# EAST-J/Dynhor

Measured on AMD Instinct MI355X. Metric: training rays/sec, higher is better.
Workload: dtype f32; 1 GPU; custom_shoes-shaped synthetic seq, 512x512, 2048 rays x (64+64) samples per rank, NeuS SDF(8x256, skip 4, softplus100) + colour(4x256) MLP, full training iteration; family=neus, frames=64, rays_per_rank=2048, samples_per_ray=128, parallelism=dp1, loss=rgb L1 + 0.1 eikonal + 0.1 mask BCE + 0.05 mono-normal

## Files before the change

### dynhor_amd/csrc/kernels_mlp_h.hip

```cpp
#include "tile.h"
#include "kernels.h"
#include "mlp_common.h"
#include "tile16h.h"
#include "workspace.h"
#include "stamps.h"

DH_STAMP_READER(dh_dev_read_stamps_h)

namespace dh {

#ifndef H2_LEAN2
#define H2_LEAN2 true
#endif

enum : int { TP_SDF_B0 = 0, TP_SDF_B8 = 8, TP_W8ROW0_T = 9, TP_W8ROW0_S = 10, TP_SCAL = 11, TP_COL_B0 = 12,
             TP_COL_W4 = 16, TP_COL_B4 = 19 };

struct SdfHPtrs {
    const u32x4* main[N_SDF];
    const u32x4* aux[N_SDF];
    const u32x4* rev[N_SDF];
    const u32x4* revaux[N_SDF];
    const float* bias[N_SDF];
    const float* w8row0;
    const float* b8_0;
    const unsigned* wabs;
};
static inline SdfHPtrs make_sdfh_ptrs(const float* packed) {
    SdfHPtrs P;
    for (int l = 0; l < N_SDF; ++l) {
        P.main[l] = reinterpret_cast<const u32x4*>(packed + PACKH.sdf_fwd_main[l]);
        P.aux[l] = reinterpret_cast<const u32x4*>(packed + PACKH.sdf_fwd_aux[l]);
        P.rev[l] = reinterpret_cast<const u32x4*>(packed + PACKH.sdf_rev_main[l]);
        P.revaux[l] = reinterpret_cast<const u32x4*>(packed + PACKH.sdf_rev_aux[l]);
        P.bias[l] = packed + PACK.sdf_bias[l];
    }
    P.w8row0 = packed + PACK.sdf_w8row0;
    P.b8_0 = packed + PACK.sdf_b8_0;
    P.wabs = reinterpret_cast<const unsigned*>(packed + PACKH.wabs);
    return P;
}
struct ColHPtrs {
    const u32x4* main[4];
    const u32x4* rev[4];
    const u32x4* aux;
    const u32x4* revaux;
    const float* bias[4];
    const float* w4;
    const float* b4;
    const unsigned* wabs;
};
static inline ColHPtrs make_colh_ptrs(const float* packed) {
    ColHPtrs C;
    for (int l = 0; l < 4; ++l) {
        C.main[l] = reinterpret_cast<const u32x4*>(packed + PACKH.col_fwd_main[l]);
        C.rev[l] = reinterpret_cast<const u32x4*>(packed + PACKH.col_rev_main[l]);
        C.bias[l] = packed + PACK.col_bias[l];
    }
    C.aux = reinterpret_cast<const u32x4*>(packed + PACKH.col_fwd_aux0);
    C.revaux = reinterpret_cast<const u32x4*>(packed + PACKH.col_rev_aux0);
    C.w4 = packed + PACK.col_w4;
    C.b4 = packed + PACK.col_b4;
    C.wabs = reinterpret_cast<const unsigned*>(packed + PACKH.wabs) + N_SDF;
    return C;
}

struct HScratch { float sred[4]; float sred2[4]; float lmax[12]; };
__device__ __forceinline__ void hs_init(HScratch& h, int tid) { if (tid < 12) h.lmax[tid] = 0.f; }
__device__ __forceinline__ TileScale lds_handoff(const f32x16 (&acc)[MT][2], _Float16* smain, HScratch& hs, float* lmax, int tid,
                                                 int wave, int lane, float extra_max = 0.f, const float* extra_lds = nullptr,
                                                 unsigned* tslot = nullptr, int sit = -1, int slayer = 0) {
    (void)sit; (void)slayer;
    tile_max_publish(hs.sred, wave, lane, acc_absmax(acc));
    DH_STAMP(sit, slayer, 3);
    __syncthreads();
    DH_STAMP(sit, slayer, 4);
    const float m = tile_max_read(hs.sred);
    if (tid == 0) {
        if (lmax) *lmax = fmaxf(*lmax, m);
        if (tslot) *tslot = __builtin_bit_cast(unsigned, m);
    }
    if (extra_lds) extra_max = fmaxf(extra_max, *extra_lds);
    const TileScale ts = scale_for_max(fmaxf(m, extra_max));
    acc_to_lds_split(acc, smain, wave, lane, ts.S);
    DH_STAMP(sit, slayer, 5);
    __syncthreads();
    DH_STAMP(sit, slayer, 6);
    return ts;
}

#ifdef DH_STAMPS
template <int KC>
__device__ __forceinline__ void gemm_stamped_steps(f32x16 (&acc)[MT][2], H2 (&a)[2][MT], H2 (&b)[4][2], const _Float16* xrow, rsrc_t wr, int woff, int it, int wave,
                                                   int lane, bool on) {
    if constexpr (KC < 16) {
        if (on) DH_STAMP(it, 5 + (KC >> 3), KC & 7);
        if constexpr (KC + 3 < 16) {
            DH_UNROLL for (int t = 0; t < 2; ++t)
                DH_UNROLL for (int p = 0; p < 2; ++p)
                    b[(KC + 3) & 3][t].p[p] = __builtin_amdgcn_raw_buffer_load_b128(wr, woff + (t * 2 + p) * 1024, (KC + 3) * (8 * 2 * 64 * 16), 0);
        }
        if constexpr (KC + 1 < 16) {
            DH_UNROLL for (int m = 0; m < MT; ++m)
                DH_UNROLL for (int p = 0; p < 2; ++p)
                    a[(KC + 1) & 1][m].p[p] = *reinterpret_cast<const u32x4*>(xrow + p * PLANE_H + m * 32 * LDH + (KC + 1) * 16);
        }
        __builtin_amdgcn_sched_barrier(0);
        mfma_only_h<0, 12>(acc, a[KC & 1], b[KC & 3]);
        __builtin_amdgcn_sched_barrier(0);
        gemm_stamped_steps<KC + 1>(acc, a, b, xrow, wr, woff, it, wave, lane, on);
    }
}
__device__ __forceinline__ void gemm_rows_stamped(f32x16 (&acc)[MT][2], const _Float16* img, const u32x4* __restrict__ wp, int wave, int lane, int it, bool on) {
    const _Float16* xrow = img + (lane & 31) * LDH + 8 * (lane >> 5);
    const rsrc_t wr = weight_rsrc(wp);
    const int woff = ((2 * wave) * 2 * 64 + lane) * 16;
    H2 a[2][MT], b[4][2];
    DH_UNROLL for (int kc = 0; kc < 3; ++kc)
        DH_UNROLL for (int t = 0; t < 2; ++t)
            DH_UNROLL for (int p = 0; p < 2; ++p)
                b[kc][t].p[p] = __builtin_amdgcn_raw_buffer_load_b128(wr, woff + (t * 2 + p) * 1024, kc * (8 * 2 * 64 * 16), 0);
    DH_UNROLL for (int m = 0; m < MT; ++m)
        DH_UNROLL for (int p = 0; p < 2; ++p) a[0][m].p[p] = *reinterpret_cast<const u32x4*>(xrow + p * PLANE_H + m * 32 * LDH);
    gemm_stamped_steps<0>(acc, a, b, xrow, wr, woff, it, wave, lane, on);
    if (on) DH_STAMP(it, 7, 0);
}
#endif

__global__ __launch_bounds__(256, 2) void color_fwd_h_kernel(ColHPtrs C, const float* __restrict__ pts, const float* __restrict__ dirs,
                                                            int n_per_ray, const float* __restrict__ normals,
                                                            const float* __restrict__ feat, int64_t npts,
                                                            float* __restrict__ color, float* __restrict__ cact,
                                                            float* __restrict__ caux, int save, unsigned* __restrict__ absmax) {
    __shared__ __attribute__((aligned(16))) _Float16 smain[IMG_H];
    __shared__ __attribute__((aligned(16))) float saux[TM * LDA];
    __shared__ HScratch hs;
    const int tid = threadIdx.x, wave = tid >> 6, lane = tid & 63;
    const int loff = tile_loff(wave, lane);
    const int64_t ntiles = (npts + TM - 1) / TM;
    hs_init(hs, tid);
    float winv[4];
    DH_UNROLL for (int l = 0; l < 4; ++l) winv[l] = winv_from_bits(C.wabs[l]);
    int it = 0;
    for (int64_t tile = blockIdx.x; tile < ntiles; tile += gridDim.x, ++it) {
        (void)it;
        if (tid < TM) {
            const int64_t gp = tile * TM + tid;
            float* row = saux + tid * LDA;
            float mx = 1.f;
            const int64_t first = tile * TM, last = first + TM - 1 < npts ? first + TM - 1 : npts - 1;
            const bool one_ray = first / n_per_ray == last / n_per_ray;
            float esin = 0.f, ecos = 0.f;
            if (one_ray && lane < 12) sincosf(dirs[(first / n_per_ray) * 3 + lane % 3] * (float)(1 << (lane / 3)), &esin, &ecos);
            if (gp < npts) {
                const int64_t ray = gp / n_per_ray;
                DH_UNROLL for (int c = 0; c < 3; ++c) {
                    const float d = dirs[ray * 3 + c], x = pts[gp * 3 + c], nn = normals[gp * 3 + c];
                    row[c] = x;
                    row[3 + c] = d;
                    DH_UNROLL for (int k = 0; k < 4; ++k) {
                        float s, co;
                        if (one_ray) {
                            s = __builtin_bit_cast(float, __builtin_amdgcn_readlane(__builtin_bit_cast(int, esin), 3 * k + c));
                            co = __builtin_bit_cast(float, __builtin_amdgcn_readlane(__builtin_bit_cast(int, ecos), 3 * k + c));
                        } else {
// ... 155 lines not shown
__global__ __launch_bounds__(256, 2) void color_bwd_h_kernel(ColHPtrs C, const float* __restrict__ colors,
                                                            const float* __restrict__ d_colors, int64_t npts,
                                                            const float* __restrict__ cact, float* __restrict__ czbar,
                                                            float* __restrict__ featbar, float* __restrict__ d_normals,
                                                            float* __restrict__ tpart, const float* __restrict__ dirs,
                                                            int n_per_ray, float* __restrict__ d_pts,
                                                            float* __restrict__ d_dirs_pts, unsigned* __restrict__ absmax,
                                                            unsigned* __restrict__ tmax) {
    __shared__ __attribute__((aligned(16))) _Float16 smain[IMG_H];
    __shared__ __attribute__((aligned(16))) float saux[TM * LDA];
    __shared__ HScratch hs;
    const int tid = threadIdx.x, wave = tid >> 6, lane = tid & 63;
    const int loff = tile_loff(wave, lane);
    const int64_t ntiles = (npts + TM - 1) / TM;
    hs_init(hs, tid);
    for (int64_t tile = blockIdx.x; tile < ntiles; tile += gridDim.x) {
        float* tp = tpart + tile * N_TILE_PART * 256;
        if (tid < TM) {
            const int64_t gp = tile * TM + tid;
            DH_UNROLL for (int j = 0; j < 3; ++j) {
                float v = 0.f;
                if (gp < npts) { const float c = colors[gp * 3 + j]; v = d_colors[gp * 3 + j] * c * (1.f - c); }
                saux[tid * 4 + j] = v;
            }
            saux[tid * 4 + 3] = 0.f;
        }
        __syncthreads();
        if (tid < 3) {
            float s = 0.f;
            for (int r = 0; r < TM; ++r) s += saux[r * 4 + tid];
            tp[TP_COL_B4 * 256 + tid] = s;
        }
        f32x16 acc[MT][2];
        acc_load_native_b(acc, tile_rsrc(cact + ((int64_t)3 * ntiles + tile) * TILE_F), loff);
        {
            const int col0 = acc_col(wave, 0, lane), col1 = acc_col(wave, 1, lane);
            float w4[3][2];
            DH_UNROLL for (int j = 0; j < 3; ++j) { w4[j][0] = C.w4[j * 256 + col0]; w4[j][1] = C.w4[j * 256 + col1]; }
            float dw[3][2] = {{0.f, 0.f}, {0.f, 0.f}, {0.f, 0.f}};
            DH_UNROLL for (int m = 0; m < MT; ++m)
                DH_UNROLL for (int r = 0; r < 16; ++r) {
                    const f32x4 cr = *reinterpret_cast<const f32x4*>(saux + acc_row(m, r, lane) * 4);
                    DH_UNROLL for (int t = 0; t < 2; ++t) {
                        const float h = acc[m][t][r];
                        DH_UNROLL for (int j = 0; j < 3; ++j) dw[j][t] = fmaf(cr[j], h, dw[j][t]);
                        const float hb = cr[0] * w4[0][t] + cr[1] * w4[1][t] + cr[2] * w4[2][t];
                        acc[m][t][r] = h > 0.f ? hb : 0.f;
                    }
                }
            DH_UNROLL for (int j = 0; j < 3; ++j)
                DH_UNROLL for (int t = 0; t < 2; ++t) {
                    float s = dw[j][t];
                    s += __shfl_xor(s, 32);
                    if (lane < 32) tp[(TP_COL_W4 + j) * 256 + 64 * wave + 32 * t + lane] = s;
                }
        }
        acc_store_native_b(acc, tile_rsrc(czbar + ((int64_t)3 * ntiles + tile) * TILE_F), loff);
        tile_colsum(acc, tp + (TP_COL_B0 + 3) * 256, wave, lane);
        TileScale ts = lds_handoff(acc, smain, hs, &hs.lmax[3], tid, wave, lane, 0.f, nullptr, tmax + (TMAX_CZBAR + 3) * ntiles + tile);
        for (int l = 3; l >= 1; --l) {
            acc_zero(acc);
            const rsrc_t hr = tile_rsrc(cact + ((int64_t)(l - 1) * ntiles + tile) * TILE_F);
            Slab h0, h1;
            gemm_rows_hp<false>(acc, smain, 16, C.rev[l], wave, lane, [&] { slab_ld(h0, hr, loff, 0); });
            slab_ld(h1, hr, loff, 1);
            const float inv = ts.inv * winv_from_bits(C.wabs[l]);
            DH_UNROLL for (int m = 0; m < MT; ++m) {
                const Slab& hs_ = m ? h1 : h0;
                DH_UNROLL for (int t = 0; t < 2; ++t)
                    DH_UNROLL for (int r4 = 0; r4 < 4; ++r4) {
                        const f32x4 h = hs_.v[t * 4 + r4];
                        DH_UNROLL for (int rr = 0; rr < 4; ++rr)
                            acc[m][t][4 * r4 + rr] = h[rr] > 0.f ? acc[m][t][4 * r4 + rr] * inv : 0.f;
                    }
                __builtin_amdgcn_sched_barrier(0);
            }
            acc_store_native_b(acc, tile_rsrc(czbar + ((int64_t)(l - 1) * ntiles + tile) * TILE_F), loff);
            tile_colsum(acc, tp + (TP_COL_B0 + l - 1) * 256, wave, lane);
            ts = lds_handoff(acc, smain, hs, &hs.lmax[l - 1], tid, wave, lane, 0.f, nullptr, tmax + (TMAX_CZBAR + l - 1) * ntiles + tile);
        }
        const float inv0 = ts.inv * winv_from_bits(C.wabs[0]);
        acc_zero(acc);
        gemm_rows_hp(acc, smain, 16, C.rev[0], wave, lane);
        acc_map(acc, [&](int, int, int, float v) { return v * inv0; });
        acc_store_native_b(acc, tile_rsrc(featbar + tile * TILE_F), loff);
        tile_max_publish(hs.sred2, wave, lane, acc_absmax(acc));
        f32x16 a2[AUX_NTW];
        aux_zero(a2);
        gemm_auxout_hp(a2, smain, 16, C.revaux, wave, lane);
        DH_UNROLL for (int tt = 0; tt < AUX_NTW; ++tt) DH_UNROLL for (int r = 0; r < 16; ++r) a2[tt][r] *= inv0;
        DH_UNROLL for (int tt = 0; tt < AUX_NTW; ++tt) {
            const int col = aux_col(wave, tt, lane);
            if (col >= 30 && col < 33) {
                DH_UNROLL for (int r = 0; r < 16; ++r) {
                    const int64_t gp = tile * TM + aux_row(wave, r, lane);
                    if (gp < npts) d_normals[gp * 3 + (col - 30)] += a2[tt][r];
                }
            }
        }
        if (RAYS) {
            __syncthreads();
            DH_UNROLL for (int tt = 0; tt < AUX_NTW; ++tt) {
                const int col = aux_col(wave, tt, lane);
                if (col < CAUX) {
                    DH_UNROLL for (int r = 0; r < 16; ++r) saux[aux_row(wave, r, lane) * LDA + col] = a2[tt][r];
                }
            }
            __syncthreads();
            if (tid < TM) {
                const int64_t gp = tile * TM + tid;
                if (gp < npts) {
                    const float* row = saux + tid * LDA;
                    const int64_t ray = gp / n_per_ray;
                    DH_UNROLL for (int c = 0; c < 3; ++c) {
                        d_pts[gp * 3 + c] = row[c];
                        const float dv = dirs[ray * 3 + c];
                        float v = row[3 + c];
                        DH_UNROLL for (int kf = 0; kf < 4; ++kf) {
                            const float f = (float)(1 << kf);
                            float sn, co; sincosf(dv * f, &sn, &co);
                            v += f * (co * row[6 + 6 * kf + c] - sn * row[6 + 6 * kf + 3 + c]);
                        }
                        d_dirs_pts[gp * 3 + c] = v;
                    }
                }
            }
        }
        __syncthreads();
        if (tid == 0) {
            const float m = tile_max_read(hs.sred2);
            hs.lmax[4] = fmaxf(hs.lmax[4], m);
            tmax[TMAX_FEATBAR * ntiles + tile] = __builtin_bit_cast(unsigned, m);
        }
    }
    if (absmax) {
        if (tid < 4) post_class_max(absmax, ABSMAX_CZBAR + tid, hs.lmax[tid]);
        if (tid == 4) post_class_max(absmax, ABSMAX_FEATBAR, hs.lmax[4]);
    }
}

__global__ __launch_bounds__(256, 2) void sdf_tangent_h_kernel(SdfHPtrs P, const float* __restrict__ pts,
                                                              const float* __restrict__ d_normals, int64_t npts,
                                                              const float* __restrict__ act, const float* __restrict__ asave,
                                                              float* __restrict__ t0aux, float* __restrict__ tsave,
                                                              float* __restrict__ rsave, float* __restrict__ tpart,
                                                              unsigned* __restrict__ absmax, unsigned* __restrict__ tmax) {
    __shared__ __attribute__((aligned(16))) _Float16 smain[IMG_H];
    __shared__ __attribute__((aligned(16))) float saux[TM * LDA];
    __shared__ HScratch hs;
    const int tid = threadIdx.x, wave = tid >> 6, lane = tid & 63;
    const int loff = tile_loff(wave, lane);
    const int64_t ntiles = (npts + TM - 1) / TM;
    hs_init(hs, tid);
    for (int64_t tile = blockIdx.x; tile < ntiles; tile += gridDim.x) {
        float* tp = tpart + tile * N_TILE_PART * 256;
        {
            const int p = tid & (TM - 1), part = tid / TM;
            const int64_t gp = tile * TM + p;
            float x[3] = {0.f, 0.f, 0.f}, nb[3] = {0.f, 0.f, 0.f};
            if (gp < npts) {
                DH_UNROLL for (int c = 0; c < 3; ++c) { x[c] = pts[gp * 3 + c]; nb[c] = d_normals[gp * 3 + c]; }
            }
            float* row = saux + p * LDA;
            float mx = 0.f;
            if (part == 0) { row[0] = nb[0]; row[1] = nb[1]; row[2] = nb[2]; mx = fmaxf(fmaxf(fabsf(nb[0]), fabsf(nb[1])), fabsf(nb[2])); }
            if (part == 1) { for (int c = 39; c < LDA; ++c) row[c] = 0.f; }
            for (int k = part; k < 6; k += TPP) {
                const float f = (float)(1 << k);
                DH_UNROLL for (int c = 0; c < 3; ++c) {
                    float s, co;
                    sincosf(x[c] * f, &s, &co);
                    const float v0 = f * co * nb[c], v1 = -f * s * nb[c];
                    row[3 + 6 * k + c] = v0;
                    row[3 + 6 * k + 3 + c] = v1;
                    mx = fmaxf(mx, fmaxf(fabsf(v0), fabsf(v1)));
                }
            }
            tile_max_publish(hs.sred2, wave, lane, wave_max(mx));
        }
        __syncthreads();
        const float m_aux = tile_max_read(hs.sred2);
        if (tid == 0) { hs.lmax[7] = fmaxf(hs.lmax[7], m_aux); tmax[TMAX_T0AUX * ntiles + tile] = __builtin_bit_cast(unsigned, m_aux); }
        const TileScale ts_aux = scale_for_max(m_aux);
        aux_lds_to_native(saux, t0aux + tile * AUXT_F, wave, lane);
        f32x16 acc[MT][2];
        TileScale ts = ts_aux;
        for (int l = 0; l < 8; ++l) {
            acc_zero(acc);
            const rsrc_t hr = tile_rsrc(act + ((int64_t)l * ntiles + tile) * TILE_F);
            const rsrc_t ar = tile_rsrc(asave + ((int64_t)l * ntiles + tile) * TILE_F);
            const rsrc_t rr_ = tile_rsrc(rsave + ((int64_t)l * ntiles + tile) * TILE_F);
            if (l > 0) gemm_rows_hp<H2_LEAN2>(acc, smain, l == 4 ? 14 : 16, P.main[l], wave, lane);
            if (l == 0 || l == 4) gemm_rows_aux_h(acc, saux, P.aux[l], wave, lane, ts.S);
            const float inv = ts.inv * winv_from_bits(P.wabs[l]);
            DH_UNROLL for (int m = 0; m < MT; ++m) {
                Slab hs_, as_;
                slab_ld(hs_, hr, loff, m); slab_ld(as_, ar, loff, m);
                DH_UNROLL for (int t = 0; t < 2; ++t)
                    DH_UNROLL for (int r4 = 0; r4 < 4; ++r4) {
                        const f32x4 h = hs_.v[t * 4 + r4], a = as_.v[t * 4 + r4];
                        f32x4 rv;
                        DH_UNROLL for (int rr = 0; rr < 4; ++rr) {
                            float s, em; softplus_deriv_from_h(h[rr], s, em);
                            const float ab = acc[m][t][4 * r4 + rr] * inv;
                            rv[rr] = ab * a[rr] * (SOFTPLUS_BETA * em);
                            acc[m][t][4 * r4 + rr] = s * ab;
                        }
                        tile_st(rr_, loff, (m * 2 + t) * 4 + r4, rv);
                    }
                __builtin_amdgcn_sched_barrier(0);
            }
            if (l < 7) {
                acc_store_native_b(acc, tile_rsrc(tsave + ((int64_t)l * ntiles + tile) * TILE_F), loff);
                ts = lds_handoff(acc, smain, hs, &hs.lmax[l], tid, wave, lane, l == 3 ? m_aux : 0.f, nullptr, tmax + (TMAX_TSAVE + l) * ntiles + tile);
            } else {
                tile_colsum(acc, tp + TP_W8ROW0_T * 256, wave, lane);
            }
        }
        __syncthreads();
    }
    if (absmax) {
        if (tid < 7) post_class_max(absmax, ABSMAX_TSAVE + tid, hs.lmax[tid]);
        if (tid == 7) post_class_max(absmax, ABSMAX_T0AUX, hs.lmax[7]);
    }
}

template <bool RAYS>
__global__ __launch_bounds__(256, 2) void sdf_bwd_h_kernel(SdfHPtrs P, const float* __restrict__ d_sdf, int64_t npts,
                                                          const float* __restrict__ act, const float* __restrict__ rsave,
                                                          const float* __restrict__ featbar, float* __restrict__ zbar,
                                                          float* __restrict__ tpart, const float* __restrict__ pts,
                                                          const float* __restrict__ d_normals, const float* __restrict__ gesave,
                                                          float* __restrict__ d_pts, unsigned* __restrict__ absmax,
                                                          unsigned* __restrict__ tmax) {
    __shared__ __attribute__((aligned(16))) _Float16 smain[IMG_H];
    __shared__ __attribute__((aligned(16))) float saux[TM * LDA];
    __shared__ HScratch hs;
    const int tid = threadIdx.x, wave = tid >> 6, lane = tid & 63;
    const int loff = tile_loff(wave, lane);
    const int64_t ntiles = (npts + TM - 1) / TM;
    hs_init(hs, tid);
    const float w0c0 = P.w8row0[acc_col(wave, 0, lane)], w0c1 = P.w8row0[acc_col(wave, 1, lane)];
    for (int64_t tile = blockIdx.x; tile < ntiles; tile += gridDim.x) {
        float* tp = tpart + tile * N_TILE_PART * 256;
        if (tid < TM) {
            const int64_t gp = tile * TM + tid;
            saux[tid] = gp < npts ? d_sdf[gp] : 0.f;
        }
        f32x16 acc[MT][2];
        f32x16 eb[AUX_NTW];
        if (RAYS) aux_zero(eb);
        acc_load_native_b(acc, tile_rsrc(featbar + tile * TILE_F), loff);
        tile_colsum(acc, tp + TP_SDF_B8 * 256, wave, lane);
        TileScale ts = lds_handoff(acc, smain, hs, nullptr, tid, wave, lane);
        if (wave == 0) {
            float s = 0.f;
            for (int i = lane; i < TM; i += 64) s += saux[i];
            DH_UNROLL for (int off = 32; off > 0; off >>= 1) s += __shfl_xor(s, off);
            if (lane == 0) tp[TP_SCAL * 256] = s;
        }
        acc_zero(acc);
        gemm_rows_hp<H2_LEAN2>(acc, smain, 16, P.rev[8], wave, lane);
        {
            const float inv = ts.inv * winv_from_bits(P.wabs[8]);
            DH_UNROLL for (int m = 0; m < MT; ++m)
                DH_UNROLL for (int r = 0; r < 16; ++r) {
                    const float sb = saux[acc_row(m, r, lane)];
                    acc[m][0][r] = fmaf(sb, w0c0, acc[m][0][r] * inv);
                    acc[m][1][r] = fmaf(sb, w0c1, acc[m][1][r] * inv);
                }
        }
        for (int l = 7; l >= 0; --l) {
            float ws0 = 0.f, ws1 = 0.f;
            DH_UNROLL for (int m = 0; m < MT; ++m) {
                Slab hs_, rs_;
                slab_ld(hs_, tile_rsrc(act + ((int64_t)l * ntiles + tile) * TILE_F), loff, m);
                slab_ld(rs_, tile_rsrc(rsave + ((int64_t)l * ntiles + tile) * TILE_F), loff, m);
                DH_UNROLL for (int t = 0; t < 2; ++t)
                    DH_UNROLL for (int r4 = 0; r4 < 4; ++r4) {
                        const f32x4 h = hs_.v[t * 4 + r4], rv = rs_.v[t * 4 + r4];
                        DH_UNROLL for (int rr = 0; rr < 4; ++rr) {
                            float s, em; softplus_deriv_from_h(h[rr], s, em);
                            if (l == 7) {
                                const float sb = saux[acc_row(m, 4 * r4 + rr, lane)];
                                if (t == 0) ws0 = fmaf(sb, h[rr], ws0); else ws1 = fmaf(sb, h[rr], ws1);
                            }
                            acc[m][t][4 * r4 + rr] = fmaf(acc[m][t][4 * r4 + rr], s, rv[rr]);
                        }
                    }
                __builtin_amdgcn_sched_barrier(0);
            }
            if (l == 7) {
                ws0 += __shfl_xor(ws0, 32); ws1 += __shfl_xor(ws1, 32);
                if (lane < 32) {
                    tp[TP_W8ROW0_S * 256 + 64 * wave + lane] = ws0;
                    tp[TP_W8ROW0_S * 256 + 64 * wave + 32 + lane] = ws1;
                }
            }
            acc_store_native_b(acc, tile_rsrc(zbar + ((int64_t)l * ntiles + tile) * TILE_F), loff);
            tile_colsum(acc, tp + (TP_SDF_B0 + l) * 256, wave, lane);
            if (l > 0) {
                ts = lds_handoff(acc, smain, hs, &hs.lmax[l], tid, wave, lane, 0.f, nullptr, tmax + (TMAX_ZBAR + l) * ntiles + tile);
                const float inv = ts.inv * winv_from_bits(P.wabs[l]);
                if (RAYS && l == 4) {
                    gemm_auxout_hp(eb, smain, 16, P.revaux[4], wave, lane);
                    DH_UNROLL for (int tt = 0; tt < AUX_NTW; ++tt) DH_UNROLL for (int r = 0; r < 16; ++r) eb[tt][r] *= inv;
                }
                acc_zero(acc);
                gemm_rows_hp<H2_LEAN2>(acc, smain, 16, P.rev[l], wave, lane);
                acc_map(acc, [&](int, int, int, float v) { return v * inv; });
            } else if (RAYS) {
                ts = lds_handoff(acc, smain, hs, &hs.lmax[0], tid, wave, lane, 0.f, nullptr, tmax + TMAX_ZBAR * ntiles + tile);
                {
                    f32x16 e0[AUX_NTW];
                    aux_zero(e0);
                    gemm_auxout_hp(e0, smain, 16, P.revaux[0], wave, lane);
                    const float inv = ts.inv * winv_from_bits(P.wabs[0]);
                    DH_UNROLL for (int tt = 0; tt < AUX_NTW; ++tt) DH_UNROLL for (int r = 0; r < 16; ++r) eb[tt][r] = fmaf(e0[tt][r], inv, eb[tt][r]);
                }
                DH_UNROLL for (int tt = 0; tt < AUX_NTW; ++tt) {
                    const int col = aux_col(wave, tt, lane);
                    if (col < AUXW) {
                        DH_UNROLL for (int r = 0; r < 16; ++r) saux[aux_row(wave, r, lane) * LDA + col] = eb[tt][r];
                    }
                }
                __syncthreads();
                if (tid < TM) {
                    const int64_t gp = tile * TM + tid;
                    if (gp < npts) {
                        const float* e = saux + tid * LDA;
                        const float* ge = gesave + gp * 40;
                        DH_UNROLL for (int c = 0; c < 3; ++c) {
                            const float x = pts[gp * 3 + c], nb = d_normals[gp * 3 + c];
                            float v = e[c], dn = 0.f;
                            DH_UNROLL for (int k = 0; k < 6; ++k) {
                                const float f = (float)(1 << k);
                                float sn, co; sincosf(x * f, &sn, &co);
                                v += f * (co * e[3 + 6 * k + c] - sn * e[3 + 6 * k + 3 + c]);
                                dn -= f * f * (sn * ge[3 + 6 * k + c] + co * ge[3 + 6 * k + 3 + c]);
                            }
                            d_pts[gp * 3 + c] += v + nb * dn;
                        }
                    }
                }
            } else {
                tile_max_publish(hs.sred2, wave, lane, acc_absmax(acc));
            }
        }
        __syncthreads();
        if (!RAYS && tid == 0) {
            const float m = tile_max_read(hs.sred2);
            hs.lmax[0] = fmaxf(hs.lmax[0], m);
            tmax[TMAX_ZBAR * ntiles + tile] = __builtin_bit_cast(unsigned, m);
        }
    }
    if (absmax && tid < 8) post_class_max(absmax, ABSMAX_ZBAR + tid, hs.lmax[tid]);
}

int launch_sdf_grad_h(const float* packed, const float* pts, int64_t npts, const float* act, float* asave, float* normals,
                      int save, float* gesave, unsigned* absmax, int grid, hipStream_t stream) {
    hipLaunchKernelGGL(sdf_grad_h_kernel, dim3(grid_for(npts, grid)), dim3(256), 0, stream, make_sdfh_ptrs(packed), pts, npts, act,
                       asave, normals, save, gesave, absmax);
    return ok();
}
int launch_color_fwd_h(const float* packed, const float* pts, const float* dirs, int n_per_ray, const float* normals,
                       const float* feat, int64_t npts, float* color, float* cact, float* caux, int save, unsigned* absmax,
                       int grid, hipStream_t stream) {
    hipLaunchKernelGGL(color_fwd_h_kernel, dim3(grid_for(npts, grid)), dim3(256), 0, stream, make_colh_ptrs(packed), pts, dirs,
                       n_per_ray, normals, feat, npts, color, cact, caux, save, absmax);
    return ok();
}
int launch_color_bwd_h(const float* packed, const float* colors, const float* d_colors, const float* dirs, int n_per_ray,
                       int64_t npts, const float* cact, float* czbar, float* featbar, float* d_normals, float* tpart,
                       float* d_pts, float* d_dirs_pts, unsigned* absmax, unsigned* tmax, int grid, hipStream_t st) {
    if (d_pts) hipLaunchKernelGGL(color_bwd_h_kernel<true>, dim3(grid_for(npts, grid)), dim3(256), 0, st, make_colh_ptrs(packed), colors,
                                  d_colors, npts, cact, czbar, featbar, d_normals, tpart, dirs, n_per_ray, d_pts, d_dirs_pts, absmax, tmax);
    else hipLaunchKernelGGL(color_bwd_h_kernel<false>, dim3(grid_for(npts, grid)), dim3(256), 0, st, make_colh_ptrs(packed), colors,
                            d_colors, npts, cact, czbar, featbar, d_normals, tpart, nullptr, 1, nullptr, nullptr, absmax, tmax);
    return ok();
}
int launch_sdf_tangent_h(const float* packed, const float* pts, const float* d_normals, int64_t npts, const float* act,
                         const float* asave, float* t0aux, float* tsave, float* rsave, float* tpart, unsigned* absmax, unsigned* tmax,
                         int grid, hipStream_t st) {
    hipLaunchKernelGGL(sdf_tangent_h_kernel, dim3(grid_for(npts, grid)), dim3(256), 0, st, make_sdfh_ptrs(packed), pts, d_normals,
                       npts, act, asave, t0aux, tsave, rsave, tpart, absmax, tmax);
    return ok();
}
int launch_sdf_bwd_h(const float* packed, const float* d_sdf, const float* pts, const float* d_normals, int64_t npts,
                     const float* act, const float* rsave, const float* featbar, const float* gesave, float* zbar, float* tpart,
                     float* d_pts, unsigned* absmax, unsigned* tmax, int grid, hipStream_t st) {
    if (d_pts) hipLaunchKernelGGL(sdf_bwd_h_kernel<true>, dim3(grid_for(npts, grid)), dim3(256), 0, st, make_sdfh_ptrs(packed), d_sdf, npts,
                                  act, rsave, featbar, zbar, tpart, pts, d_normals, gesave, d_pts, absmax, tmax);
    else hipLaunchKernelGGL(sdf_bwd_h_kernel<false>, dim3(grid_for(npts, grid)), dim3(256), 0, st, make_sdfh_ptrs(packed), d_sdf, npts,
                            act, rsave, featbar, zbar, tpart, nullptr, nullptr, nullptr, nullptr, absmax, tmax);
    return ok();
}

}
```

### dynhor_amd/csrc/tile16h.h

```cpp
#pragma once
#include "tile16.h"
#include "workspace.h"

namespace dh {

typedef _Float16 f16x8 __attribute__((ext_vector_type(8)));
typedef _Float16 f16x2v __attribute__((ext_vector_type(2)));
struct H2 { u32x4 p[2]; };
__device__ __forceinline__ unsigned pack_f16x2(f32x2 v) { return __builtin_bit_cast(unsigned, __builtin_convertvector(v, f16x2v)); }
__device__ __forceinline__ f32x2 resid_f16x2(f32x2 v, unsigned h) {
    f32x2 r;
#ifdef H2_VISIBLE_RESID
    const f16x2v hv = __builtin_bit_cast(f16x2v, h);
    r[0] = v[0] - (float)hv[0];
    r[1] = v[1] - (float)hv[1];
#else
    asm("v_fma_mix_f32 %0, -%1, 1.0, %2 op_sel_hi:[1,0,0]" : "=v"(r[0]) : "v"(h), "v"(v[0]));
    asm("v_fma_mix_f32 %0, -%1, 1.0, %2 op_sel:[1,0,0] op_sel_hi:[1,0,0]" : "=v"(r[1]) : "v"(h), "v"(v[1]));
#endif
    return r;
}
__device__ __forceinline__ f32x16 mfma_h(const u32x4& a, const u32x4& b, const f32x16& c) {
    return __builtin_amdgcn_mfma_f32_32x32x16_f16(__builtin_bit_cast(f16x8, a), __builtin_bit_cast(f16x8, b), c, 0, 0, 0);
}
// ... 37 lines not shown
    t.inv = __builtin_bit_cast(float, pow2_inv_bits(sb));
    return t;
}
template <int CTRL, int ROW_MASK>
__device__ __forceinline__ float wave_max_step(float m) {
    const int o = __builtin_amdgcn_update_dpp(0, __builtin_bit_cast(int, m), CTRL, ROW_MASK, 0xf, false);
    return fmaxf(m, __builtin_bit_cast(float, o));
}
__device__ __forceinline__ float wave_max(float m) {
#ifdef DH_WAVE_MAX_SHFL
    DH_UNROLL for (int off = 32; off > 0; off >>= 1) m = fmaxf(m, __shfl_xor(m, off));
    return m;
#endif
    m = wave_max_step<0x111, 0xf>(m);
    m = wave_max_step<0x112, 0xf>(m);
    m = wave_max_step<0x114, 0xf>(m);
    m = wave_max_step<0x118, 0xf>(m);
    m = wave_max_step<0x142, 0xa>(m);
    m = wave_max_step<0x143, 0xc>(m);
    return __builtin_bit_cast(float, __builtin_amdgcn_readlane(__builtin_bit_cast(int, m), 63));
}
__device__ __forceinline__ float acc_absmax(const f32x16 (&acc)[MT][2]) {
    float m0 = 0.f, m1 = 0.f;
    DH_UNROLL for (int m = 0; m < MT; ++m)
        DH_UNROLL for (int t = 0; t < 2; ++t)
            DH_UNROLL for (int r = 0; r < 16; r += 2) { m0 = fmaxf(m0, fabsf(acc[m][t][r])); m1 = fmaxf(m1, fabsf(acc[m][t][r + 1])); }
    return wave_max(fmaxf(m0, m1));
}
__device__ __forceinline__ void tile_max_publish(float* sred, int wave, int lane, float m) { if (lane == 0) sred[wave] = m; }
__device__ __forceinline__ float tile_max_read(const float* sred) { return fmaxf(fmaxf(sred[0], sred[1]), fmaxf(sred[2], sred[3])); }
__device__ __forceinline__ TileScale tile_scale(const float* sred, float* lmax, int tid) {
    const float m = tile_max_read(sred);
    if (lmax && tid == 0) *lmax = fmaxf(*lmax, m);
    return scale_for_max(m);
}
__device__ __forceinline__ void post_class_max(unsigned* absmax, int cls, float m) {
    atomicMax(absmax + cls * ABSMAX_STRIDE, __builtin_bit_cast(unsigned, m));
}
__device__ __forceinline__ unsigned watch_max3(unsigned m, float a, float b) {
    return max(m, max(__builtin_bit_cast(unsigned, a), __builtin_bit_cast(unsigned, b)));
}
__device__ __forceinline__ float watch_close(unsigned m) { return __builtin_bit_cast(float, min(m, 0x7f800000u)); }
constexpr int LDH = 264;
constexpr int PLANE_H = TM * LDH;
constexpr int IMG_H = 2 * PLANE_H;
__device__ __forceinline__ void acc_to_lds_split(const f32x16 (&acc)[MT][2], _Float16* img, int wave, int lane, float S) {
    DH_UNROLL for (int m = 0; m < MT; ++m)
        DH_UNROLL for (int t = 0; t < 2; ++t) {
            _Float16* base = img + (m * 32 + 4 * (lane >> 5)) * LDH + acc_col(wave, t, lane);
            DH_UNROLL for (int r = 0; r < 16; r += 2) {
                f32x2 x;
                x[0] = acc[m][t][r] * S;
                x[1] = acc[m][t][r + 1] * S;
                const unsigned h = pack_f16x2(x);
                const unsigned l = pack_f16x2(resid_f16x2(x, h));
                const f16x2v hv = __builtin_bit_cast(f16x2v, h), lv = __builtin_bit_cast(f16x2v, l);
                _Float16* q = base + ((r & 3) + 8 * (r >> 2)) * LDH;
                q[0] = hv[0]; q[LDH] = hv[1];
                q[PLANE_H] = lv[0]; q[PLANE_H + LDH] = lv[1];
#ifdef H_PROBE_EXTRA_WRITES
                asm volatile("ds_write_b16 %0, %1 offset:%2\n\tds_write_b16_d16_hi %0, %1 offset:%3" ::"v"((unsigned)(uintptr_t)q), "v"(l), "n"(PLANE_H * 2), "n"((PLANE_H + LDH) * 2) : "memory");
#endif
            }
        }
}
struct SplitStateH { f32x2 r[4 * MT]; float sc; };
template <int STEP, bool SC>
__device__ __forceinline__ void split_step_h(H2 (&a)[MT], const RawA& raw, SplitStateH& st) {
    constexpr int j = STEP / 3, s = STEP % 3, m = j / 4, q = j % 4;
    if constexpr (s == 0) {
        f32x2 x;
        x[0] = q < 2 ? raw.lo[m][2 * q] : raw.hi[m][2 * q - 4];
        x[1] = q < 2 ? raw.lo[m][2 * q + 1] : raw.hi[m][2 * q - 3];
        if constexpr (SC) { x[0] *= st.sc; x[1] *= st.sc; }
        a[m].p[0][q] = pack_f16x2(x);
        st.r[j] = x;
    } else if constexpr (s == 1) {
        st.r[j] = resid_f16x2(st.r[j], a[m].p[0][q]);
    } else {
        a[m].p[1][q] = pack_f16x2(st.r[j]);
    }
}

template <int I>
__device__ __forceinline__ void mfma_step_h(f32x16 (&acc)[MT][2], const H2 (&a)[MT], const H2 (&b)[2]) {
    constexpr int pa[3] = {0, 1, 0}, pb[3] = {1, 0, 0};
    constexpr int p = I / (2 * MT), mt = I % (2 * MT), m = mt / 2, t = mt % 2;
    acc[m][t] = mfma_h(a[m].p[pa[p]], b[t].p[pb[p]], acc[m][t]);
}
template <int I, int N>
__device__ __forceinline__ void mfma_only_h(f32x16 (&acc)[MT][2], const H2 (&ac)[MT], const H2 (&bc)[2]) {
    if constexpr (I < N) { mfma_step_h<I>(acc, ac, bc); mfma_only_h<I + 1, N>(acc, ac, bc); }
}

typedef __amdgpu_buffer_rsrc_t rsrc_t;
__device__ __forceinline__ rsrc_t tile_rsrc(const float* tile) {
    return __builtin_amdgcn_make_buffer_rsrc(const_cast<float*>(tile), 0, TILE_F * 4, 0x00020000);
}
__device__ __forceinline__ int tile_loff(int wave, int lane) { return (wave * MT * 8 * 64 + lane) * 16; }
__device__ __forceinline__ f32x4 tile_ld(rsrc_t r, int loff, int idx) {
    const int off = idx * 1024;
    return __builtin_bit_cast(f32x4, __builtin_amdgcn_raw_buffer_load_b128(r, loff + (off & 4095), off & ~4095, 2));
}
__device__ __forceinline__ void tile_st(rsrc_t r, int loff, int idx, const f32x4& v) {
    __builtin_amdgcn_raw_buffer_store_b128(__builtin_bit_cast(u32x4, v), r, loff + idx * 1024, 0, 2);
}
__device__ __forceinline__ void acc_store_native_b(const f32x16 (&acc)[MT][2], rsrc_t r, int loff) {
    DH_UNROLL for (int m = 0; m < MT; ++m)
        DH_UNROLL for (int t = 0; t < 2; ++t)
            DH_UNROLL for (int r4 = 0; r4 < 4; ++r4) {
                f32x4 v;
                v[0] = acc[m][t][4 * r4 + 0]; v[1] = acc[m][t][4 * r4 + 1]; v[2] = acc[m][t][4 * r4 + 2]; v[3] = acc[m][t][4 * r4 + 3];
                tile_st(r, loff, (m * 2 + t) * 4 + r4, v);
            }
}
__device__ __forceinline__ void acc_load_native_b(f32x16 (&acc)[MT][2], rsrc_t r, int loff) {
    DH_UNROLL for (int m = 0; m < MT; ++m)
        DH_UNROLL for (int t = 0; t < 2; ++t)
            DH_UNROLL for (int r4 = 0; r4 < 4; ++r4) {
                const f32x4 v = tile_ld(r, loff, (m * 2 + t) * 4 + r4);
                acc[m][t][4 * r4 + 0] = v[0]; acc[m][t][4 * r4 + 1] = v[1]; acc[m][t][4 * r4 + 2] = v[2]; acc[m][t][4 * r4 + 3] = v[3];
            }
}
struct Slab { f32x4 v[8]; };
__device__ __forceinline__ void slab_ld(Slab& s, rsrc_t r, int loff, int m) {
    DH_UNROLL for (int i = 0; i < 8; ++i) s.v[i] = tile_ld(r, loff, m * 8 + i);
}
__device__ __forceinline__ rsrc_t weight_rsrc(const u32x4* wp) {
    return __builtin_amdgcn_make_buffer_rsrc(const_cast<u32x4*>(wp), 0, 0x40000000, 0x00020000);
}

struct NoPre { __device__ __forceinline__ void operator()() const {} };
template <bool LEAN = false, class Pre = NoPre>
__device__ __forceinline__ void gemm_rows_hp(f32x16 (&acc)[MT][2], const _Float16* img, const int nkc,
                                             const u32x4* __restrict__ wp, const int wave, const int lane, Pre&& pre = Pre()) {
    static_assert(MT == 2, "");
    const _Float16* xrow = img + (lane & 31) * LDH + 8 * (lane >> 5);
    const rsrc_t wr = weight_rsrc(wp);
    const int woff = ((2 * wave) * 2 * 64 + lane) * 16;
    auto loadb = [&](H2 (&b)[2], int kc) {
        DH_UNROLL for (int t = 0; t < 2; ++t)
            DH_UNROLL for (int p = 0; p < 2; ++p)
                b[t].p[p] = __builtin_amdgcn_raw_buffer_load_b128(wr, woff + (t * 2 + p) * 1024, kc * (8 * 2 * 64 * 16), 0);
    };
    auto loada = [&](H2 (&a)[MT], int kc) {
        DH_UNROLL for (int m = 0; m < MT; ++m)
            DH_UNROLL for (int p = 0; p < 2; ++p)
                a[m].p[p] = *reinterpret_cast<const u32x4*>(xrow + p * PLANE_H + m * 32 * LDH + kc * 16);
    };
    H2 a0[MT], a1[MT];
    if constexpr (LEAN) {
        H2 b0[2], b1[2];
        loadb(b0, 0); loada(a0, 0);
        _Pragma("unroll 1") for (int kc = 0; kc < nkc; kc += 2) {
            loadb(b1, kc + 1); loada(a1, kc + 1);
            __builtin_amdgcn_sched_barrier(0);
            mfma_only_h<0, 12>(acc, a0, b0);
            __builtin_amdgcn_sched_barrier(0);
            if (kc + 2 < nkc) { loadb(b0, kc + 2); loada(a0, kc + 2); }
            else pre();
            __builtin_amdgcn_sched_barrier(0);
            mfma_only_h<0, 12>(acc, a1, b1);
            __builtin_amdgcn_sched_barrier(0);
        }
        return;
    }
    H2 bA[2], bB[2], bC[2], bD[2];
    auto step2 = [&](int c, H2 (&b0)[2], H2 (&b1)[2], H2 (&b2)[2], H2 (&b3)[2]) {
        loadb(b2, c + 2); loada(a1, c + 1);
        __builtin_amdgcn_sched_barrier(0);
        mfma_only_h<0, 12>(acc, a0, b0);
        __builtin_amdgcn_sched_barrier(0);
        loadb(b3, c + 3); loada(a0, c + 2);
        __builtin_amdgcn_sched_barrier(0);
        mfma_only_h<0, 12>(acc, a1, b1);
        __builtin_amdgcn_sched_barrier(0);
    };
    auto tail4 = [&](int c, H2 (&b0)[2], H2 (&b1)[2], H2 (&b2)[2], H2 (&b3)[2]) {
        loadb(b2, c + 2); loada(a1, c + 1);
        __builtin_amdgcn_sched_barrier(0);
        mfma_only_h<0, 12>(acc, a0, b0);
        __builtin_amdgcn_sched_barrier(0);
        loadb(b3, c + 3);
        pre();
        loada(a0, c + 2);
        __builtin_amdgcn_sched_barrier(0);
        mfma_only_h<0, 12>(acc, a1, b1);
        __builtin_amdgcn_sched_barrier(0);
        loada(a1, c + 3);
        __builtin_amdgcn_sched_barrier(0);
        mfma_only_h<0, 12>(acc, a0, b2);
        __builtin_amdgcn_sched_barrier(0);
        mfma_only_h<0, 12>(acc, a1, b3);
        __builtin_amdgcn_sched_barrier(0);
    };
    loadb(bA, 0); loadb(bB, 1); loada(a0, 0);
    int kc = 0;
    _Pragma("unroll 1") for (; kc + 8 <= nkc; kc += 4) {
        step2(kc, bA, bB, bC, bD);
        step2(kc + 2, bC, bD, bA, bB);
    }
    if (nkc - kc == 6) {
        step2(kc, bA, bB, bC, bD);
        tail4(kc + 2, bC, bD, bA, bB);
    } else {
        tail4(kc, bA, bB, bC, bD);
    }
}

__device__ __forceinline__ void gemm_rows_aux_h(f32x16 (&acc)[MT][2], const float* xs, const u32x4* __restrict__ wp,
                                                const int wave, const int lane, const float sc) {
    static_assert(AUX_KC == 3, "");
    const float* xrow = xs + (lane & 31) * LDA + 8 * (lane >> 5);
    const rsrc_t wr = weight_rsrc(wp);
    const int woff = ((2 * wave) * 2 * 64 + lane) * 16;
    H2 b[AUX_KC][2];
    asm volatile("" ::: "memory");
    DH_UNROLL for (int kc = 0; kc < AUX_KC; ++kc)
        DH_UNROLL for (int t = 0; t < 2; ++t)
            DH_UNROLL for (int p = 0; p < 2; ++p)
                b[kc][t].p[p] = __builtin_amdgcn_raw_buffer_load_b128(wr, woff + (t * 2 + p) * 1024, kc * (8 * 2 * 64 * 16), 0);
    DH_UNROLL for (int kc = 0; kc < AUX_KC; ++kc) {
        H2 a[MT];
        DH_UNROLL for (int m = 0; m < MT; ++m) {
            const f32x4 lo = *reinterpret_cast<const f32x4*>(xrow + m * 32 * LDA + kc * 16);
            const f32x4 hi = *reinterpret_cast<const f32x4*>(xrow + m * 32 * LDA + kc * 16 + 4);
            a[m] = split2(lo * sc, hi * sc);
        }
        mfma_only_h<0, 12>(acc, a, b[kc]);
    }
}

__device__ __forceinline__ void gemm_auxout_hp(f32x16 (&acc2)[AUX_NTW], const _Float16* img, const int nkc,
                                               const u32x4* __restrict__ wp, const int wave, const int lane) {
    const _Float16* xrow = img + (32 * aux_mtile(wave) + (lane & 31)) * LDH + 8 * (lane >> 5);
    const rsrc_t wr = weight_rsrc(wp);
    const int woff = (aux_ntile(wave, 0) * 2 * 64 + lane) * 16;
    const int last = nkc - 1;
    auto fetch = [&](H2& a, H2 (&b)[AUX_NTW], int kc) {
        kc = kc < last ? kc : last;
        DH_UNROLL for (int t = 0; t < AUX_NTW; ++t)
            DH_UNROLL for (int p = 0; p < 2; ++p)
                b[t].p[p] = __builtin_amdgcn_raw_buffer_load_b128(wr, woff + (t * 2 + p) * 1024, kc * (2 * 2 * 64 * 16), 0);
        DH_UNROLL for (int p = 0; p < 2; ++p) a.p[p] = *reinterpret_cast<const u32x4*>(xrow + p * PLANE_H + kc * 16);
    };
    H2 a0, a1, b0[AUX_NTW], b1[AUX_NTW];
    fetch(a0, b0, 0);
    _Pragma("unroll 1") for (int kc = 0; kc < nkc; kc += 2) {
        fetch(a1, b1, kc + 1);
        DH_UNROLL for (int t = 0; t < AUX_NTW; ++t) acc2[t] = mfma3(a0, b0[t], acc2[t]);
        if (kc + 1 < nkc) {
            fetch(a0, b0, kc + 2);
            DH_UNROLL for (int t = 0; t < AUX_NTW; ++t) acc2[t] = mfma3(a1, b1[t], acc2[t]);
        }
    }
}

__device__ __forceinline__ float row_dot256_hp(const _Float16* img, const float* __restrict__ w, int tid) {
    constexpr int TPP_ = 256 / TM, SEG = 256 / TPP_;
    const int p = tid / TPP_, part = tid % TPP_;
    const f16x8* xh = reinterpret_cast<const f16x8*>(img + p * LDH + part * SEG);
    const f16x8* xl = reinterpret_cast<const f16x8*>(img + PLANE_H + p * LDH + part * SEG);
    const f32x4* wr = reinterpret_cast<const f32x4*>(w + part * SEG);
    float s = 0.f;
    DH_UNROLL for (int i = 0; i < SEG / 8; ++i) {
        const f16x8 h = xh[i], l = xl[i];
        const f32x4 b0 = wr[2 * i], b1 = wr[2 * i + 1];
        DH_UNROLL for (int j = 0; j < 4; ++j) s = fmaf((float)h[j] + (float)l[j], b0[j], s);
        DH_UNROLL for (int j = 0; j < 4; ++j) s = fmaf((float)h[4 + j] + (float)l[4 + j], b1[j], s);
    }
    DH_UNROLL for (int off = 1; off < TPP_; off <<= 1) s += __shfl_xor(s, off);
    return s;
}

}
```

Before: 235,600 rays/s.

## Prefetch epilogue slabs during GEMM tail and recompute last-layer tangent activation

Issues the epilogue's act/asave/rsave slab loads from inside the final GEMM iteration via the pre() hook, and requests the second m-slab before the first is processed. This lets global-memory latency overlap the tail MFMAs. The tangent kernel's last layer now recomputes the activation from w8row0*softplus instead of loading asave, and skips a dead aux GEMM. The backward loop is restructured so each layer's GEMM sits next to its epilogue. The costs are higher register pressure from holding two slabs, and rounding may change slightly where contraction is disabled and values are recomputed.

Result: no change. 238,200 rays/s, median of 6 (+1.1%).

```diff
diff --git a/dynhor_amd/csrc/kernels_mlp_h.hip b/dynhor_amd/csrc/kernels_mlp_h.hip
--- a/dynhor_amd/csrc/kernels_mlp_h.hip
+++ b/dynhor_amd/csrc/kernels_mlp_h.hip
@@ -4,6 +4,7 @@
 #include "tile16h.h"
 #include "workspace.h"
 #include "stamps.h"
+#include <type_traits>
 
 DH_STAMP_READER(dh_dev_read_stamps_h)
 
@@ -11,6 +12,15 @@
 
 #ifndef H2_LEAN2
 #define H2_LEAN2 true
+#endif
+#ifndef H2_TAIL_PRE
+#define H2_TAIL_PRE true
+#endif
+#ifndef H2_EPI_PIPE
+#define H2_EPI_PIPE true
+#endif
+#ifndef H2_TAN_A7
+#define H2_TAN_A7 true
 #endif
 
 enum : int { TP_SDF_B0 = 0, TP_SDF_B8 = 8, TP_W8ROW0_T = 9, TP_W8ROW0_S = 10, TP_SCAL = 11, TP_COL_B0 = 12,
@@ -472,6 +482,7 @@
     const int loff = tile_loff(wave, lane);
     const int64_t ntiles = (npts + TM - 1) / TM;
     hs_init(hs, tid);
+    const float w8c0 = P.w8row0[acc_col(wave, 0, lane)], w8c1 = P.w8row0[acc_col(wave, 1, lane)];
     for (int64_t tile = blockIdx.x; tile < ntiles; tile += gridDim.x) {
         float* tp = tpart + tile * N_TILE_PART * 256;
         {
@@ -505,38 +516,53 @@
         aux_lds_to_native(saux, t0aux + tile * AUXT_F, wave, lane);
         f32x16 acc[MT][2];
         TileScale ts = ts_aux;
-        for (int l = 0; l < 8; ++l) {
+        auto layer = [&](const int l, auto last) {
+            constexpr bool LAST = decltype(last)::value, OWN_A = LAST && H2_TAN_A7;
             acc_zero(acc);
             const rsrc_t hr = tile_rsrc(act + ((int64_t)l * ntiles + tile) * TILE_F);
             const rsrc_t ar = tile_rsrc(asave + ((int64_t)l * ntiles + tile) * TILE_F);
             const rsrc_t rr_ = tile_rsrc(rsave + ((int64_t)l * ntiles + tile) * TILE_F);
-            if (l > 0) gemm_rows_hp<H2_LEAN2>(acc, smain, l == 4 ? 14 : 16, P.main[l], wave, lane);
-            if (l == 0 || l == 4) gemm_rows_aux_h(acc, saux, P.aux[l], wave, lane, ts.S);
+            Slab hs_[MT], as_[MT];
+            auto request = [&](int m) { slab_ld(hs_[m], hr, loff, m); if constexpr (!OWN_A) slab_ld(as_[m], ar, loff, m); };
+            if (l > 0) {
+                if constexpr (H2_TAIL_PRE) gemm_rows_hp<H2_LEAN2>(acc, smain, l == 4 ? 14 : 16, P.main[l], wave, lane, [&] { request(0); });
+                else gemm_rows_hp<H2_LEAN2>(acc, smain, l == 4 ? 14 : 16, P.main[l], wave, lane);
+            }
+            if (!LAST && (l == 0 || l == 4)) gemm_rows_aux_h(acc, saux, P.aux[l], wave, lane, ts.S);
             const float inv = ts.inv * winv_from_bits(P.wabs[l]);
+            if (!H2_TAIL_PRE || l == 0) request(0);
+            if constexpr (H2_EPI_PIPE) { request(1); __builtin_amdgcn_sched_barrier(0); }
             DH_UNROLL for (int m = 0; m < MT; ++m) {
-                Slab hs_, as_;
-                slab_ld(hs_, hr, loff, m); slab_ld(as_, ar, loff, m);
+                if constexpr (!H2_EPI_PIPE) { if (m > 0) request(m); }
                 DH_UNROLL for (int t = 0; t < 2; ++t)
                     DH_UNROLL for (int r4 = 0; r4 < 4; ++r4) {
-                        const f32x4 h = hs_.v[t * 4 + r4], a = as_.v[t * 4 + r4];
+                        const f32x4 h = hs_[m].v[t * 4 + r4];
+                        f32x4 a;
+                        if constexpr (!OWN_A) a = as_[m].v[t * 4 + r4];
                         f32x4 rv;
                         DH_UNROLL for (int rr = 0; rr < 4; ++rr) {
                             float s, em; softplus_deriv_from_h(h[rr], s, em);
+                            if constexpr (OWN_A) a[rr] = (t ? w8c1 : w8c0) * s;
                             const float ab = acc[m][t][4 * r4 + rr] * inv;
                             rv[rr] = ab * a[rr] * (SOFTPLUS_BETA * em);
-                            acc[m][t][4 * r4 + rr] = s * ab;
+                            {
+#pragma clang fp contract(off)
+                                acc[m][t][4 * r4 + rr] = s * ab;
+                            }
                         }
                         tile_st(rr_, loff, (m * 2 + t) * 4 + r4, rv);
                     }
                 __builtin_amdgcn_sched_barrier(0);
             }
-            if (l < 7) {
+            if constexpr (!LAST) {
                 acc_store_native_b(acc, tile_rsrc(tsave + ((int64_t)l * ntiles + tile) * TILE_F), loff);
                 ts = lds_handoff(acc, smain, hs, &hs.lmax[l], tid, wave, lane, l == 3 ? m_aux : 0.f, nullptr, tmax + (TMAX_TSAVE + l) * ntiles + tile);
             } else {
                 tile_colsum(acc, tp + TP_W8ROW0_T * 256, wave, lane);
             }
-        }
+        };
+        for (int l = 0; l < 7; ++l) layer(l, std::false_type());
+        layer(7, std::true_type());
         __syncthreads();
     }
     if (absmax) {
@@ -579,38 +605,53 @@
             DH_UNROLL for (int off = 32; off > 0; off >>= 1) s += __shfl_xor(s, off);
             if (lane == 0) tp[TP_SCAL * 256] = s;
         }
-        acc_zero(acc);
-        gemm_rows_hp<H2_LEAN2>(acc, smain, 16, P.rev[8], wave, lane);
-        {
-            const float inv = ts.inv * winv_from_bits(P.wabs[8]);
-            DH_UNROLL for (int m = 0; m < MT; ++m)
-                DH_UNROLL for (int r = 0; r < 16; ++r) {
-                    const float sb = saux[acc_row(m, r, lane)];
-                    acc[m][0][r] = fmaf(sb, w0c0, acc[m][0][r] * inv);
-                    acc[m][1][r] = fmaf(sb, w0c1, acc[m][1][r] * inv);
-                }
-        }
         for (int l = 7; l >= 0; --l) {
+            const float inv = ts.inv * winv_from_bits(P.wabs[l + 1]);
+            if (RAYS && l == 3) {
+                gemm_auxout_hp(eb, smain, 16, P.revaux[4], wave, lane);
+                DH_UNROLL for (int tt = 0; tt < AUX_NTW; ++tt) DH_UNROLL for (int r = 0; r < 16; ++r) eb[tt][r] *= inv;
+            }
+            Slab hs_[MT], rs_[MT];
+            auto request = [&](int m) {
+                slab_ld(hs_[m], tile_rsrc(act + ((int64_t)l * ntiles + tile) * TILE_F), loff, m);
+                slab_ld(rs_[m], tile_rsrc(rsave + ((int64_t)l * ntiles + tile) * TILE_F), loff, m);
+            };
+            acc_zero(acc);
+            if constexpr (H2_TAIL_PRE) gemm_rows_hp<H2_LEAN2>(acc, smain, 16, P.rev[l + 1], wave, lane, [&] { request(0); });
+            else gemm_rows_hp<H2_LEAN2>(acc, smain, 16, P.rev[l + 1], wave, lane);
+            if (l == 7) {
+                DH_UNROLL for (int m = 0; m < MT; ++m)
+                    DH_UNROLL for (int r = 0; r < 16; ++r) {
+                        const float sb = saux[acc_row(m, r, lane)];
+                        acc[m][0][r] = fmaf(sb, w0c0, acc[m][0][r] * inv);
+                        acc[m][1][r] = fmaf(sb, w0c1, acc[m][1][r] * inv);
+                    }
+            } else {
+                acc_map(acc, [&](int, int, int, float v) { return v * inv; });
+            }
             float ws0 = 0.f, ws1 = 0.f;
+            if constexpr (!H2_TAIL_PRE) request(0);
+            if constexpr (H2_EPI_PIPE) { request(1); __builtin_amdgcn_sched_barrier(0); }
             DH_UNROLL for (int m = 0; m < MT; ++m) {
-                Slab hs_, rs_;
-                slab_ld(hs_, tile_rsrc(act + ((int64_t)l * ntiles + tile) * TILE_F), loff, m);
-                slab_ld(rs_, tile_rsrc(rsave + ((int64_t)l * ntiles + tile) * TILE_F), loff, m);
+                if constexpr (!H2_EPI_PIPE) { if (m > 0) request(m); }
                 DH_UNROLL for (int t = 0; t < 2; ++t)
                     DH_UNROLL for (int r4 = 0; r4 < 4; ++r4) {
-                        const f32x4 h = hs_.v[t * 4 + r4], rv = rs_.v[t * 4 + r4];
+                        const f32x4 h = hs_[m].v[t * 4 + r4], rv = rs_[m].v[t * 4 + r4];
                         DH_UNROLL for (int rr = 0; rr < 4; ++rr) {
                             float s, em; softplus_deriv_from_h(h[rr], s, em);
-                            if (l == 7) {
-                                const float sb = saux[acc_row(m, 4 * r4 + rr, lane)];
-                                if (t == 0) ws0 = fmaf(sb, h[rr], ws0); else ws1 = fmaf(sb, h[rr], ws1);
-                            }
                             acc[m][t][4 * r4 + rr] = fmaf(acc[m][t][4 * r4 + rr], s, rv[rr]);
                         }
                     }
                 __builtin_amdgcn_sched_barrier(0);
             }
             if (l == 7) {
+                DH_UNROLL for (int m = 0; m < MT; ++m)
+                    DH_UNROLL for (int r4 = 0; r4 < 4; ++r4)
+                        DH_UNROLL for (int rr = 0; rr < 4; ++rr) {
+                            const float sb = saux[acc_row(m, 4 * r4 + rr, lane)];
+                            ws0 = fmaf(sb, hs_[m].v[r4][rr], ws0);
+                            ws1 = fmaf(sb, hs_[m].v[4 + r4][rr], ws1);
+                        }
                 ws0 += __shfl_xor(ws0, 32); ws1 += __shfl_xor(ws1, 32);
                 if (lane < 32) {
                     tp[TP_W8ROW0_S * 256 + 64 * wave + lane] = ws0;
@@ -621,14 +662,6 @@
             tile_colsum(acc, tp + (TP_SDF_B0 + l) * 256, wave, lane);
             if (l > 0) {
                 ts = lds_handoff(acc, smain, hs, &hs.lmax[l], tid, wave, lane, 0.f, nullptr, tmax + (TMAX_ZBAR + l) * ntiles + tile);
-                const float inv = ts.inv * winv_from_bits(P.wabs[l]);
-                if (RAYS && l == 4) {
-                    gemm_auxout_hp(eb, smain, 16, P.revaux[4], wave, lane);
-                    DH_UNROLL for (int tt = 0; tt < AUX_NTW; ++tt) DH_UNROLL for (int r = 0; r < 16; ++r) eb[tt][r] *= inv;
-                }
-                acc_zero(acc);
-                gemm_rows_hp<H2_LEAN2>(acc, smain, 16, P.rev[l], wave, lane);
-                acc_map(acc, [&](int, int, int, float v) { return v * inv; });
             } else if (RAYS) {
                 ts = lds_handoff(acc, smain, hs, &hs.lmax[0], tid, wave, lane, 0.f, nullptr, tmax + TMAX_ZBAR * ntiles + tile);
                 {
diff --git a/dynhor_amd/csrc/tile16h.h b/dynhor_amd/csrc/tile16h.h
--- a/dynhor_amd/csrc/tile16h.h
+++ b/dynhor_amd/csrc/tile16h.h
@@ -213,17 +213,24 @@
     if constexpr (LEAN) {
         H2 b0[2], b1[2];
         loadb(b0, 0); loada(a0, 0);
-        _Pragma("unroll 1") for (int kc = 0; kc < nkc; kc += 2) {
+        _Pragma("unroll 1") for (int kc = 0; kc + 2 < nkc; kc += 2) {
             loadb(b1, kc + 1); loada(a1, kc + 1);
             __builtin_amdgcn_sched_barrier(0);
             mfma_only_h<0, 12>(acc, a0, b0);
             __builtin_amdgcn_sched_barrier(0);
-            if (kc + 2 < nkc) { loadb(b0, kc + 2); loada(a0, kc + 2); }
-            else pre();
+            loadb(b0, kc + 2); loada(a0, kc + 2);
             __builtin_amdgcn_sched_barrier(0);
             mfma_only_h<0, 12>(acc, a1, b1);
             __builtin_amdgcn_sched_barrier(0);
         }
+        loadb(b1, nkc - 1); loada(a1, nkc - 1);
+        __builtin_amdgcn_sched_barrier(0);
+        mfma_only_h<0, 12>(acc, a0, b0);
+        __builtin_amdgcn_sched_barrier(0);
+        pre();
+        __builtin_amdgcn_sched_barrier(0);
+        mfma_only_h<0, 12>(acc, a1, b1);
+        __builtin_amdgcn_sched_barrier(0);
         return;
     }
     H2 bA[2], bB[2], bC[2], bD[2];
```
